# yukiteruono/pbsim3

Measured on AMD Instinct MI355X. Metric: simulated bases/sec, higher is better.
Workload: dtype u8

## Files before the change

pbsim3_amd/csrc/ctx.h:

```cpp
#pragma once
#include <hip/hip_runtime.h>
#include <limits.h>
#include <stdio.h>
#include <stdlib.h>
#include <stdint.h>

#include <algorithm>
#include <condition_variable>
#include <functional>
#include <memory>
#include <mutex>
#include <string>
#include <vector>

#include "../../include/pbsim3_amd.h"
#include "host_tables.h"
#include "kernels.h"

namespace pbsim {
extern thread_local std::string g_err;
int fail(const std::string &m);
}


// ... 55 lines not shown
      return e;
    }
    bytes = want;
    return hipSuccess;
  }
};

using namespace pbsim;

constexpr int kMaxSlots = 6;
constexpr int kPipelineDepth = 2;
static_assert(kPipelineDepth >= 1 && kPipelineDepth <= kMaxSlots, "the pipeline's slots are the first of kMaxSlots");

constexpr size_t kScratchSlack = 64u << 10;
constexpr double kSinkBatchBases = 5.0e9;

constexpr int kDfBuffers = 5;
struct DfLane {
  DevBuf d_df_status, d_df_ctl;
  uint32_t epoch = 0;
  DevBuf d_df_dense[kDfBuffers];
  DevBuf d_df_code;
  HostBuf h_df_total, h_df_out[kDfBuffers];
  hipStream_t stream = nullptr;
  hipStream_t copy_stream = nullptr;
  bool own_streams = false;
  hipStream_t own[2] = {nullptr, nullptr};
  bool pre_valid = false, pre_own_staging = false, pre_elsewhere = false;
  const uint8_t *pre_text = nullptr;
  int64_t pre_n = 0;
  int pre_count = 0;
  hipStream_t lane_stream = nullptr;
  hipEvent_t ev_pre = nullptr;
  hipEvent_t ev_df[kDfBuffers] = {}, ev_cp[kDfBuffers] = {};
  hipEvent_t ev_k0[kDfBuffers] = {}, ev_k1[kDfBuffers] = {};
  std::vector<std::unique_ptr<HostBuf>> arena_blocks;
  std::vector<size_t> arena_fill;
  std::vector<char> arena_touched;
  std::vector<int> arena_idle;
  std::vector<std::pair<const char *, int64_t>> arena_segs;
  size_t arena_bytes() const {
    size_t n = 0;
    for (const auto &b : arena_blocks) n += b->bytes;
    return n;
  }
  void arena_reset() {
    std::fill(arena_fill.begin(), arena_fill.end(), 0);
    arena_segs.clear();
  }
  char *arena_reserve(int64_t n, size_t max_bytes) {
    static const size_t kBlock = getenv("PBSIM_PINNED_BLOCK_KB") && atoll(getenv("PBSIM_PINNED_BLOCK_KB")) > 0
                                     ? (size_t)atoll(getenv("PBSIM_PINNED_BLOCK_KB")) << 10 : (size_t)256u << 20;
    const size_t need = ((size_t)n + 63) & ~(size_t)63;
    for (size_t i = 0; i < arena_blocks.size(); i++) {
      HostBuf &b = *arena_blocks[i];
      if (arena_fill[i] + need <= b.bytes) {
        char *p = (char *)b.p + arena_fill[i];
        arena_fill[i] += need;
        arena_touched[i] = 1;
        arena_segs.emplace_back(p, n);
        return p;
      }
    }
    const size_t want = std::max(kBlock, need);
    if (max_bytes && arena_bytes() + want > max_bytes) return nullptr;
    if (getenv("PBSIM_TRACE")) fprintf(stderr, "[pbsim arena] new block of %zu MB (lane holds %zu MB in %zu blocks)\n", want >> 20, arena_bytes() >> 20, arena_blocks.size());
// ... 208 lines not shown
  hipEvent_t ev_prof_base = nullptr;
  std::vector<std::pair<float, float>> prof_intervals;
  double prof_text_ms = 0, prof_deflate_ms = 0;
  int64_t prof_text_launches = 0, prof_text_in = 0, prof_text_out = 0;
  int64_t prof_deflate_launches = 0, prof_deflate_in = 0, prof_deflate_out = 0;
  std::mutex prof_mu;
};

namespace pbsim {
RefDesc current_ref(const pbsim_ctx *c);
int64_t quota_of(const pbsim_ctx *c, int64_t ref_len);
int walk_begin(pbsim_ctx *c, const RefDesc &ref, int64_t first_read, int64_t n_reads, int64_t truncate_remaining, bool chain = false,
               double factor = 0.0 );
double scratch_factor_of(const pbsim_ctx *c);
int chain_end_finalize(pbsim_ctx *c, int64_t len_total_before, pbsim_batch_info *out);
int chain_reads_for(const pbsim_ctx *c, int64_t ref_len, int64_t remaining);
constexpr int kChainReads = 6;
int64_t batch_capacity_for(const pbsim_ctx *c, int64_t ref_len);
int finalize_cut(pbsim_ctx *c, int64_t len_total_before, pbsim_batch_info *out);
int finalize_text(pbsim_ctx *c, pbsim_batch_info *info);
int finalize_uncut(pbsim_ctx *c, pbsim_batch_info *out);
std::string sam_header_text(const pbsim_ctx *c, int64_t unit);
std::string truth_bam_header_bytes(const pbsim_ctx *c, int64_t ref_len);
int truth_bam_check_names(const pbsim_ctx *c);
int account_slot(pbsim_ctx *c, StatsAcc *st);
int account_of(pbsim_ctx *c, Slot &sl, StatsAcc *st);
void stats_add_task(StatsAcc *st, int64_t len_max, bool quality, long len, long nsub, long nins, long ndel, double qsum,
                    std::vector<double> *values);
void stats_finish(const StatsAcc &st, const pbsim_params &p, int64_t ref_len, pbsim_stats *o);
int stats_merge(StatsAcc *st, const pbsim_params &p, const pbsim_comm *comm, int64_t *extra, int n_extra);
int deflate_prelaunch(pbsim_ctx *c, Slot &sl, bool want_read, bool want_maf);
int deflate_pieces(pbsim_ctx *c, DfLane &lane, const uint8_t *d_text, int64_t n,
                   const std::function<int(const char *, int64_t)> &consume,
                   const std::function<char *(int64_t)> *place = nullptr);
int ensure_deflate_ready(pbsim_ctx *c);
int ensure_crc_tables(pbsim_ctx *c);
int prepare_enqueue(pbsim_ctx *c, uint8_t *d_seq, DevBuf &hp, DevBuf &tiles, DevBuf &flags, int64_t len, hipStream_t stream);
int ensure_tables(pbsim_ctx *c, bool hp11);
inline bool has_quality(const pbsim_ctx *c) { return c->p.method == PBSIM_METHOD_QS || c->p.method == PBSIM_METHOD_SAMPLE; }
}
```

pbsim3_amd/csrc/deflate_host.cpp:

```cpp
#include <hip/hip_runtime.h>
#include <limits.h>
#include <math.h>
#include <stdio.h>
#include <stdlib.h>
#include <string.h>

#include <algorithm>
#include <chrono>
#include <functional>
#include <memory>
#include <string>
#include <thread>
#include <vector>

#include "ctx.h"
#include "engine_internal.h"
#include "unit_io.h"

extern "C" {

extern "C++" {
namespace {

int ensure_deflate_tables(pbsim_ctx *c) {
// ... 76 lines not shown
  launch_deflate_table(d_text, n, reinterpret_cast<uint32_t *>(sl.d_df_code.as<uint8_t>() + DF_TABLE_BYTES), sl.d_df_code.p, sl.stream);
  if (!sl.ev_df[0]) {
    for (int i = 0; i < kDfBuffers; i++) {
      HIP_OK(hipEventCreateWithFlags(&sl.ev_df[i], hipEventDisableTiming));
      HIP_OK(hipEventCreateWithFlags(&sl.ev_cp[i], hipEventDisableTiming));
      HIP_OK(hipEventCreate(&sl.ev_k0[i]));
      HIP_OK(hipEventCreate(&sl.ev_k1[i]));
    }
  }
  unsigned long long *d_prof = nullptr;
  if (getenv("PBSIM_DEFLATE_PROF")) {
    HIP_OK(c->d_df_prof.ensure(128));
    HIP_OK(hipMemsetAsync(c->d_df_prof.p, 0, 128, sl.stream));
    d_prof = c->d_df_prof.as<unsigned long long>();
  }
  const int64_t first = std::min<int64_t>(launch_stream ? 1 : g.ahead, g.n_pieces);
  for (int64_t j = 0; j < first; j++)
    if (!df_launch_piece(c, sl, g, d_text, n, j, false, own_staging, d_prof)) return PBSIM_FAILED;
  sl.pre_count = (int)first;
  sl.pre_text = d_text;
  sl.pre_n = n;
  sl.pre_own_staging = own_staging;
  sl.pre_valid = true;
  sl.pre_elsewhere = launch_stream != nullptr;
  if (launch_stream) {
    if (!sl.ev_pre) HIP_OK(hipEventCreateWithFlags(&sl.ev_pre, hipEventDisableTiming));
    HIP_OK(hipEventRecord(sl.ev_pre, launch_stream));
  }
  return PBSIM_SUCCEEDED;
}

template <class F>
int deflate_stream(pbsim_ctx *c, DfLane &sl, const uint8_t *d_text, int64_t n, F &&consume,
                   const std::function<char *(int64_t)> *place = nullptr) {
  if (n <= 0) return PBSIM_SUCCEEDED;
  const bool prelaunched = sl.pre_valid && sl.pre_text == d_text && sl.pre_n == n && sl.pre_own_staging == (place == nullptr);
  sl.pre_valid = false;
  if (!prelaunched && !df_begin(c, sl, d_text, n, place == nullptr, nullptr)) return PBSIM_FAILED;
  sl.pre_valid = false;
  if (sl.pre_elsewhere) {
    sl.stream = sl.lane_stream;
    HIP_OK(hipStreamWaitEvent(sl.stream, sl.ev_pre, 0));
    sl.pre_elsewhere = false;
  }
  const DfGeom g = df_geom(n);
  const int64_t n_pieces = g.n_pieces;
  const int ahead = g.ahead, nbuf = g.nbuf;
  unsigned long long *d_prof = getenv("PBSIM_DEFLATE_PROF") ? c->d_df_prof.as<unsigned long long>() : nullptr;
  const bool trace = getenv("PBSIM_DEFLATE_TRACE") != nullptr;
  const auto now = []() { return std::chrono::duration<double, std::milli>(std::chrono::steady_clock::now().time_since_epoch()).count(); };
  double t_kernel = 0, t_copy = 0, t_consume = 0, t_begin = now();
  int64_t out_bytes = 0;
  std::vector<std::pair<hipEvent_t, hipEvent_t>> tev;
  bool used[kDfBuffers] = {false};
  int64_t *h_total = reinterpret_cast<int64_t *>(sl.h_df_total.p);
  auto launch = [&](int64_t j) -> int {
    return df_launch_piece(c, sl, g, d_text, n, j, used[(int)(j % nbuf)], place == nullptr, d_prof);
  };
  for (int64_t j = sl.pre_count; j < std::min<int64_t>(ahead, n_pieces); j++)
    if (!launch(j)) return PBSIM_FAILED;
  const char *prev_ptr = nullptr;
  int64_t prev_bytes = 0;
  int prev_buf = 0;
  for (int64_t k = 0; k < n_pieces; k++) {
    const int b = (int)(k % nbuf);
    const double t0 = now();
    HIP_OK(hipEventSynchronize(sl.ev_df[b]));
    t_kernel += now() - t0;
    const int64_t total = h_total[2 * b + 1];
    if ((uint64_t)h_total[2 * b] >> 32) return fail("deflate: a workgroup's look-back gave up waiting for its predecessors");
    out_bytes += total;
    {
      float ms = 0;
      if (hipEventElapsedTime(&ms, sl.ev_k0[b], sl.ev_k1[b]) == hipSuccess) {
        std::lock_guard<std::mutex> lk(c->prof_mu);
        c->prof_deflate_ms += ms;
        c->prof_deflate_launches++;
        c->prof_deflate_in += g.len(k, n);
        c->prof_deflate_out += total;
      }
    }
    char *dst = place ? (*place)(total) : (char *)sl.h_df_out[b].p;
    if (!dst) return fail("deflate: no room for a compressed piece");
    HIP_OK(hipStreamWaitEvent(sl.copy_stream, sl.ev_df[b], 0));
    if (trace) {
      hipEvent_t e0 = nullptr, e1 = nullptr;
      HIP_OK(hipEventCreate(&e0));
      HIP_OK(hipEventCreate(&e1));
      tev.emplace_back(e0, e1);
      HIP_OK(hipEventRecord(e0, sl.copy_stream));
    }
    HIP_OK(hipMemcpyAsync(dst, sl.d_df_dense[b].p, (size_t)total, hipMemcpyDeviceToHost, sl.copy_stream));
    if (trace) HIP_OK(hipEventRecord(tev.back().second, sl.copy_stream));
    HIP_OK(hipEventRecord(sl.ev_cp[b], sl.copy_stream));
    used[b] = true;
    if (prev_bytes) {
      const double t1 = now();
      HIP_OK(hipEventSynchronize(sl.ev_cp[prev_buf]));
      const double t2 = now();
      if (!consume(prev_ptr, prev_bytes)) return PBSIM_FAILED;
      t_copy += t2 - t1;
      t_consume += now() - t2;
    }
    prev_ptr = dst;
    prev_bytes = total;
    prev_buf = b;
    if (k + ahead < n_pieces && !launch(k + ahead)) return PBSIM_FAILED;
  }
  if (prev_bytes) {
    const double t1 = now();
    HIP_OK(hipEventSynchronize(sl.ev_cp[prev_buf]));
    const double t2 = now();
    if (!consume(prev_ptr, prev_bytes)) return PBSIM_FAILED;
    t_copy += t2 - t1;
    t_consume += now() - t2;
  }
  if (trace) {
    double t_link = 0, t_span = 0;
    float ms = 0;
    for (auto &e : tev) {
      if (hipEventElapsedTime(&ms, e.first, e.second) == hipSuccess) t_link += ms;
    }
    if (!tev.empty() && hipEventElapsedTime(&ms, tev.front().first, tev.back().second) == hipSuccess) t_span = ms;
    for (auto &e : tev) {
      (void)hipEventDestroy(e.first);
      (void)hipEventDestroy(e.second);
    }
    fprintf(stderr,
            "[deflate] %.1f MB -> %.1f MB in %.1f ms: waited %.1f ms for kernels, %.1f ms for copies, %.1f ms in the consumer; copies: "
            "%.1f ms on the engine within a span of %.1f ms (%.1f GB/s while copying)\n",
            n / 1e6, out_bytes / 1e6, now() - t_begin, t_kernel, t_copy, t_consume, t_link, t_span, t_link > 0 ? out_bytes / t_link / 1e6 : 0.0);
  }
  if (d_prof) {
    unsigned long long t[16];
    HIP_OK(hipMemcpy(t, d_prof, 128, hipMemcpyDeviceToHost));
    const double nch = (double)((n + DF_CHUNK - 1) / DF_CHUNK);
    static const char *names[7] = {"stage", "crc", "sizes+scan", "header", "tokens", "trailer", "store"};
    fprintf(stderr, "[deflate prof] %.0f chunks; us per chunk (lane 0):", nch);
    for (int i = 0; i < 7; ++i) fprintf(stderr, " %s %.1f", names[i], t[i] / nch / 100);
    fprintf(stderr, "\n");
  }
  return PBSIM_SUCCEEDED;
}

int deflate_to_host(pbsim_ctx *c, DfLane &sl, const uint8_t *d_text, int64_t n, char *host_dst, int64_t cap,
                    int64_t *out_bytes) {
  int64_t written = 0;
  const int ok = deflate_stream(c, sl, d_text, n, [&](const char *z, int64_t k) {
    if (written + k > cap) return fail("deflate: output buffer too small");
    memcpy(host_dst + written, z, (size_t)k);
    written += k;
    return PBSIM_SUCCEEDED;
  });
  *out_bytes = written;
  return ok;
}

}
}

extern "C++" int pbsim::deflate_pieces(pbsim_ctx *c, DfLane &lane, const uint8_t *d_text, int64_t n,
                                       const std::function<int(const char *, int64_t)> &consume,
                                       const std::function<char *(int64_t)> *place) {
  return deflate_stream(c, lane, d_text, n, consume, place);
}
extern "C++" int pbsim::ensure_deflate_ready(pbsim_ctx *c) {
  for (auto &lane : c->df_streams)
    for (hipStream_t &st : lane)
      if (!st) HIP_OK(hipStreamCreateWithFlags(&st, hipStreamNonBlocking));
  return ensure_deflate_tables(c);
}
extern "C++" int pbsim::ensure_crc_tables(pbsim_ctx *c) { return ensure_deflate_tables(c); }
extern "C++" int pbsim::deflate_prelaunch(pbsim_ctx *c, Slot &sl, bool want_read, bool want_maf) {
  const pbsim_batch_info &bi = sl.b_info;
  if (want_read && bi.read_text_bytes > 0 && !df_begin(c, sl.df[0], sl.d_read_text.as<uint8_t>(), bi.read_text_bytes, true, sl.stream))
    return PBSIM_FAILED;
  if (want_maf && bi.maf_text_bytes > 0 && !df_begin(c, sl.df[1], sl.d_maf_text.as<uint8_t>(), bi.maf_text_bytes, true, sl.stream))
    return PBSIM_FAILED;
  return PBSIM_SUCCEEDED;
}

int pbsim_set_deflate(pbsim_ctx *c, int on) {
  if (!c) return fail("bad argument");
  c->deflate = on & 3;
  c->deflate_parallel = (on & 4) != 0;
  return PBSIM_SUCCEEDED;
}

int64_t pbsim_deflate_bound(int64_t n) {
  if (n <= 0) return 0;
  return n + ((n + DF_CHUNK - 1) / DF_CHUNK) * 31;
}

int pbsim_batch_fetch_deflated(pbsim_ctx *c, char *read_gz, int64_t read_cap, char *maf_gz, int64_t maf_cap,
                               int64_t *read_gz_bytes, int64_t *maf_gz_bytes) {
  if (!c || !c->s().b_finalized) return fail("pbsim_batch_fetch_deflated: no finalized batch");
  NEED_DEVICE(c);
// ... 93 lines not shown
```

pbsim3_amd/csrc/engine.cpp:

```cpp
#include <hip/hip_runtime.h>
#include <limits.h>
#include <math.h>
#include <stdio.h>
#include <stdlib.h>
#include <string.h>

#include <algorithm>
#include <chrono>
#include <functional>
#include <memory>
#include <string>
#include <thread>
#include <unordered_map>
#include <vector>

#include "ctx.h"
#include "engine_internal.h"
#include "unit_io.h"
#include "philox.h"

namespace pbsim {
thread_local std::string g_err;
int fail(const std::string &m) {
  g_err = m;
// ... 234 lines not shown
    (void)hipEventCreate(&sl.ev2);
    (void)hipEventCreate(&sl.ev3);
  }
  if (const char *sf = getenv("PBSIM_SCRATCH_FACTOR")) {
    if (atof(sf) >= 1.0) {
      c->scratch_factor = std::min(2.0, atof(sf));
      c->scratch_factor_fixed = true;
    }
  }
  const char *mb = getenv("PBSIM_SCRATCH_MB");
  c->scratch_budget = (mb && atoll(mb) > 0) ? atoll(mb) * (1LL << 20) : (8LL << 30);
  c->scratch_auto = !(mb && atoll(mb) > 0);
  return c.release();
}

void pbsim_destroy(pbsim_ctx *c) {
  if (!c) return;
  if (c->device >= 0) (void)hipSetDevice(c->device);
  if (c->stream) (void)hipStreamSynchronize(c->stream);
  for (Slot &sl : c->slots) {
    if (sl.stream) (void)hipStreamSynchronize(sl.stream);
    if (sl.ev0) (void)hipEventDestroy(sl.ev0);
    if (sl.ev1) (void)hipEventDestroy(sl.ev1);
    if (sl.ev2) (void)hipEventDestroy(sl.ev2);
    if (sl.ev3) (void)hipEventDestroy(sl.ev3);
    if (sl.stream) (void)hipStreamDestroy(sl.stream);
    for (DfLane &L : sl.df) {
      for (int i = 0; i < kDfBuffers; i++) {
        if (L.ev_df[i]) (void)hipEventDestroy(L.ev_df[i]);
        if (L.ev_cp[i]) (void)hipEventDestroy(L.ev_cp[i]);
        if (L.ev_k0[i]) (void)hipEventDestroy(L.ev_k0[i]);
        if (L.ev_k1[i]) (void)hipEventDestroy(L.ev_k1[i]);
      }
      for (hipStream_t &st : L.own)
        if (st) (void)hipStreamDestroy(st);
    }
    if (sl.walk_stream) (void)hipStreamDestroy(sl.walk_stream);
    if (sl.ev_prep) (void)hipEventDestroy(sl.ev_prep);
    if (sl.coop_stream) (void)hipStreamDestroy(sl.coop_stream);
    if (sl.ev_coop) (void)hipEventDestroy(sl.ev_coop);
    if (sl.ev_text) (void)hipEventDestroy(sl.ev_text);
    if (sl.ev_t0) (void)hipEventDestroy(sl.ev_t0);
    if (sl.ev_c0) (void)hipEventDestroy(sl.ev_c0);
    if (sl.ev_c1) (void)hipEventDestroy(sl.ev_c1);
    if (sl.ev_t1) (void)hipEventDestroy(sl.ev_t1);
  }
  for (auto &lane : c->df_streams)
    for (hipStream_t &st : lane)
      if (st) (void)hipStreamDestroy(st);
  if (c->ev_prof_base) (void)hipEventDestroy(c->ev_prof_base);
  if (c->prefetch_stream) (void)hipStreamDestroy(c->prefetch_stream);
  if (c->sq_stream) (void)hipStreamDestroy(c->sq_stream);
  for (Slot &sl : c->slots) {
    if (sl.ev_sq_walk) (void)hipEventDestroy(sl.ev_sq_walk);
    if (sl.ev_sq_done) (void)hipEventDestroy(sl.ev_sq_done);
  }
  if (c->stream) (void)hipStreamDestroy(c->stream);
  delete c;
}

int pbsim_load_errhmm(pbsim_ctx *c, const char *path) {
  if (!c || !path) return fail("pbsim_load_errhmm: bad argument");
  std::unique_ptr<ErrModel> m(new ErrModel);
  std::string e;
  if (!parse_errhmm(path, m.get(), &e)) return fail(e);
  c->err = std::move(m);
  c->class_tables_dirty = true;
  c->coop_wg_errhmm[0] = c->coop_wg_errhmm[1] = 0;
  return PBSIM_SUCCEEDED;
}

int pbsim_load_qshmm(pbsim_ctx *c, const char *path) {
  if (!c || !path) return fail("pbsim_load_qshmm: bad argument");
  std::unique_ptr<QsModel> m(new QsModel);
  std::string e;
  if (!parse_qshmm(path, m.get(), &e)) return fail(e);
  c->qs = std::move(m);
  c->class_tables_dirty = true;
  c->coop_wg_errhmm[0] = c->coop_wg_errhmm[1] = 0;
  return PBSIM_SUCCEEDED;
}

int pbsim_release_pools(pbsim_ctx *c) {
  if (!c) return fail("bad argument");
  NEED_DEVICE(c);
  HIP_OK(hipSetDevice(c->device));
  for (Slot &sl : c->slots) {
    if (sl.b_enqueued) return fail("pbsim_release_pools: a batch is in flight");
    if (sl.stream) HIP_OK(hipStreamSynchronize(sl.stream));
  }
  HIP_OK(hipDeviceSynchronize());
  for (Slot &sl : c->slots) {
    sl.d_scratch.release();
    sl.d_read_text.release();
    sl.d_maf_text.release();
    for (DfLane &L : sl.df) {
      for (DevBuf &b : L.d_df_dense) b.release();
      L.arena_release();
    }
    sl.b_walked = sl.b_finalized = false;
  }
  {
    std::lock_guard<std::mutex> lk(c->job_mu);
    c->job_spare.clear();
  }
  return PBSIM_SUCCEEDED;
}

int pbsim_set_scratch_bytes(pbsim_ctx *c, int64_t bytes) {
  if (!c || bytes < (1 << 20)) return fail("pbsim_set_scratch_bytes: bad argument");
  c->scratch_budget = bytes;
  c->scratch_auto = false;
  return PBSIM_SUCCEEDED;
}

int pbsim_add_hp_census(pbsim_ctx *c, const uint8_t *seq, int64_t len) {
  if (!c || !seq || len < 1) return fail("pbsim_add_hp_census: bad argument");
  NEED_DEVICE(c);
  HIP_OK(hipSetDevice(c->device));
  HIP_OK(c->d_seq_own.ensure((size_t)len + 64));
  HIP_OK(hipMemcpyAsync(c->d_seq_own.p, seq, (size_t)len, hipMemcpyHostToDevice, c->stream));
  HIP_OK(hipMemsetAsync(c->d_seq_own.as<uint8_t>() + len, 0, 64, c->stream));
// ... 1201 lines not shown
```

pbsim3_amd/csrc/job.cpp:

```cpp
#include <math.h>
#include <stdio.h>
#include <stdlib.h>
#include <string.h>

#include <algorithm>
#include <atomic>
#include <chrono>
#include <condition_variable>
#include <deque>
#include <future>
#include <mutex>
#include <thread>

#include "ctx.h"

using namespace pbsim;

namespace {

double now_us() {
  return std::chrono::duration<double, std::micro>(std::chrono::steady_clock::now().time_since_epoch()).count();
}

constexpr double kMinBatchBases = 2.0e9;
constexpr int kRoundsPerRecord = 4;

struct Rec {
  RefDesc ref;
  int64_t quota = 0, len_total = 0, next_read = 1, spec_read = 1;
  double spec_total = 0;
  int64_t cap = 0;
  bool bulk_done = false;
  bool done = false;
  int owner = -1;
  int tail_slot = -1;
  bool tail_waiting = false;
  int64_t read_off = 0, maf_off = 0;
  int64_t tail_read = 0, tail_maf = 0;
  StatsAcc st;
  bool merged = false;
};

struct Round {
  int rec, slot;
  int64_t first, n_per;
  double mean;
  bool clear;
// ... 248 lines not shown
      if (r.slot == s) return true;
    for (const Rec &r : recs)
      if (r.tail_slot == s) return true;
    return false;
  }
  static constexpr int kTailSlot = kMaxSlots - 2;
  int free_slot() const {
    for (int s = 0; s < kTailSlot; s++)
      if (!slot_busy(s)) return s;
    return -1;
  }
  int free_tail_slot() const {
    for (int s = kTailSlot; s < kMaxSlots; s++)
      if (!slot_busy(s)) return s;
    return -1;
  }
  int bulk_in_flight() const { return (int)fifo.size(); }
  int acquire_slot() {
    const double t0 = now_us();
    for (;;) {
      const int s = free_slot();
      if (s >= 0) {
        bd_slot_wait += now_us() - t0;
        return s;
      }
      std::unique_lock<std::mutex> lk(worker.mu);
      worker.cv_idle.wait_for(lk, std::chrono::milliseconds(2));
    }
  }

  void drop_round(const Round &r) {
    c->cur = r.slot;
    (void)hipStreamSynchronize(c->s().stream);
    c->s().b_enqueued = false;
  }
  void drop_rounds_of(int rec) {
    for (auto it = fifo.begin(); it != fifo.end();) {
      if (it->rec == rec) {
        drop_round(*it);
        it = fifo.erase(it);
      } else {
        ++it;
      }
    }
  }
  void drop_everything(bool failing = true) {
    if (failing) {
      giving_up = true;
      { std::lock_guard<std::mutex> lk(out_mu); }
      out_cv.notify_all();
    }
    worker.drain();
    tail_worker.drain();
    for (const Round &r : fifo) drop_round(r);
    fifo.clear();
    for (Rec &r : recs)
      if (r.tail_slot >= 0) {
        c->cur = r.tail_slot;
        (void)hipStreamSynchronize(c->s().stream);
        c->s().b_enqueued = false;
        r.tail_slot = -1;
      }
  }

  size_t arena_max = 0;
  bool wants_text() const { return sink && (sink->on_read_text || sink->on_maf_text); }
  bool deflated() const { return wants_text() && c->deflate == 3; }

  int fetch_plain(Slot &sl) {
    const pbsim_batch_info &bi = sl.b_info;
    const bool want_r = sink->on_read_text && bi.read_text_bytes, want_m = sink->on_maf_text && bi.maf_text_bytes;
    if (want_r) {
      HIP_OK(sl.h_read_text.ensure((size_t)bi.read_text_bytes + 16));
      HIP_OK(hipMemcpyAsync(sl.h_read_text.p, sl.d_read_text.p, (size_t)bi.read_text_bytes, hipMemcpyDeviceToHost, sl.stream));
    }
    if (want_m) {
      HIP_OK(sl.h_maf_text.ensure((size_t)bi.maf_text_bytes + 16));
      HIP_OK(hipMemcpyAsync(sl.h_maf_text.p, sl.d_maf_text.p, (size_t)bi.maf_text_bytes, hipMemcpyDeviceToHost, sl.stream));
    }
    HIP_OK(hipStreamSynchronize(sl.stream));
    return PBSIM_SUCCEEDED;
  }
  int call_sink(int which, int64_t unit, const char *text, int64_t bytes, int64_t at) {
    std::lock_guard<std::mutex> lk(sink_mu[which]);
    return (which == 0 ? sink->on_read_text : sink->on_maf_text)(sink->user, unit, text, bytes, at);
  }
  int sink_plain(Slot &sl, int64_t unit, int64_t read_at, int64_t maf_at) {
    const pbsim_batch_info &bi = sl.b_info;
    if (sink->on_read_text && bi.read_text_bytes && !call_sink(0, unit, (const char *)sl.h_read_text.p, bi.read_text_bytes, read_at))
      return fail("sink aborted (read text)");
    if (sink->on_maf_text && bi.maf_text_bytes && !call_sink(1, unit, (const char *)sl.h_maf_text.p, bi.maf_text_bytes, maf_at))
      return fail("sink aborted (MAF text)");
    return PBSIM_SUCCEEDED;
  }
  template <class F>
  int both_lanes(Slot &sl, F &&lane) {
    const pbsim_batch_info &bi = sl.b_info;
    if (c->deflate_parallel && bi.read_text_bytes && bi.maf_text_bytes && sink->on_read_text && sink->on_maf_text) {
      int ok_read = PBSIM_SUCCEEDED;
      std::string err_read;
      std::thread t([&]() {
        (void)hipSetDevice(c->device);
        ok_read = lane(0);
        if (!ok_read) err_read = g_err;
      });
      const int ok_maf = lane(1);
      t.join();
      if (!ok_read) return fail(err_read);
      return ok_maf;
    }
    return lane(0) && lane(1);
  }
  int stream_deflated(Slot &sl, int64_t unit, int64_t read_at, int64_t maf_at, int64_t *read_gz, int64_t *maf_gz) {
    const pbsim_batch_info &bi = sl.b_info;
    *read_gz = *maf_gz = 0;
    return both_lanes(sl, [&](int which) -> int {
      const bool is_read = which == 0;
      const int64_t n = is_read ? bi.read_text_bytes : bi.maf_text_bytes;
      auto cb = is_read ? sink->on_read_text : sink->on_maf_text;
      int64_t *sent = is_read ? read_gz : maf_gz;
      const int64_t base = is_read ? read_at : maf_at;
      const uint8_t *d = is_read ? sl.d_read_text.as<uint8_t>() : sl.d_maf_text.as<uint8_t>();
      if (!cb || n == 0) return PBSIM_SUCCEEDED;
      return deflate_pieces(c, sl.df[which], d, n, [&](const char *z, int64_t k) {
        if (!call_sink(which, unit, z, k, base + *sent)) return fail(is_read ? "sink aborted (read text)" : "sink aborted (MAF text)");
        *sent += k;
        return PBSIM_SUCCEEDED;
      });
    });
  }
  int arena_fill(Slot &sl, int64_t *read_gz, int64_t *maf_gz) {
    const pbsim_batch_info &bi = sl.b_info;
    *read_gz = *maf_gz = 0;
    return both_lanes(sl, [&](int which) -> int {
      DfLane &L = sl.df[which];
      L.arena_reset();
      const int64_t n = which == 0 ? bi.read_text_bytes : bi.maf_text_bytes;
      auto cb = which == 0 ? sink->on_read_text : sink->on_maf_text;
      if (!cb || n == 0) return PBSIM_SUCCEEDED;
      const uint8_t *d = which == 0 ? sl.d_read_text.as<uint8_t>() : sl.d_maf_text.as<uint8_t>();
      bool oom = false;
      const std::function<char *(int64_t)> place = [&](int64_t k) -> char * {
        char *p = L.arena_reserve(k, arena_max);
        if (!p) oom = true;
        return p;
      };
      if (!deflate_pieces(c, L, d, n, [](const char *, int64_t) { return PBSIM_SUCCEEDED; }, &place))
        return oom ? fail("out of pinned host memory for a compressed batch (PBSIM_PINNED_ARENA_MB bounds a lane's arena)") : PBSIM_FAILED;
      int64_t tot = 0;
      for (const auto &sg : L.arena_segs) tot += sg.second;
      (which == 0 ? *read_gz : *maf_gz) = tot;
      return PBSIM_SUCCEEDED;
    });
  }
  int arena_flush(Slot &sl, int64_t unit, int64_t read_at, int64_t maf_at) {
    return both_lanes(sl, [&](int which) -> int {
      int64_t at = which == 0 ? read_at : maf_at;
      for (const auto &sg : sl.df[which].arena_segs) {
        if (!call_sink(which, unit, sg.first, sg.second, at)) return fail(which == 0 ? "sink aborted (read text)" : "sink aborted (MAF text)");
        at += sg.second;
      }
      sl.df[which].arena_segs.clear();
      return PBSIM_SUCCEEDED;
    });
  }

  void submit_stage1(Delivery *d) {
    d->stage1 = std::make_shared<std::promise<int>>();
    d->stage1_done = d->stage1->get_future();
    if (!d->mine) {
      d->stage1->set_value(PBSIM_SUCCEEDED);
      return;
    }
    delivering[d->slot] = true;
    Slot *sl = &c->slots[d->slot];
    Rec *R = &recs[(size_t)d->rec];
    auto prom = d->stage1;
    int64_t *sizes = d->sizes;
    const int64_t read_at = R->read_off, maf_at = R->maf_off;
    std::atomic<int> *out = &rec_out[(size_t)d->rec], *bulk = &rec_bulk[(size_t)d->rec];
// ... 249 lines not shown
    const double t0 = now_us();
    progress(4, rec);
    if (!stats_merge(&R.st, c->p, multi ? comm : nullptr, extra, 3)) return PBSIM_FAILED;
    bd_merge += now_us() - t0;
    if (!tail_ok) return fail(tail_err);
    if (!check_worker()) return PBSIM_FAILED;
    if (extra[2]) {
      peer_failed = true;
      return fail("another rank of the job failed");
    }
    R.merged = R.done = true;
    pbsim_stats st;
    stats_finish(R.st, c->p, R.ref.len, &st);
    c->st = R.st;
    c->st.blocks.clear();
    R.st = StatsAcc();
    if (sink && sink->on_record_done &&
        !sink->on_record_done(sink->user, recs[(size_t)rec].ref.unit, &st, R.read_off + extra[0], R.maf_off + extra[1]))
      return fail("sink aborted (record done)");
    return PBSIM_SUCCEEDED;
  }

  int begin_round(int rec) {
    Rec &R = recs[(size_t)rec];
    const double remaining = (double)R.quota - R.spec_total;
    int64_t n_total = (int64_t)(1.005 * remaining / mean) + 64;
    if (remaining <= 0) n_total = 64;
    int64_t n_per = std::min<int64_t>((n_total + W - 1) / W, R.cap);
    if (rounds < 2) n_per = std::min<int64_t>(n_per, std::max<int64_t>(64, (int64_t)((double)R.cap * (rounds == 0 ? 0.2 : 0.5))));
    n_per = std::max<int64_t>(n_per, 1);
    if (!collect(rec)) return PBSIM_FAILED;
    const int s = acquire_slot();
    c->cur = s;
    const double tb = now_us();
    if (trace) fprintf(stderr, "[pbsim job r%d] begin rec %d first=%lld n_per=%lld\n", rank, rec + 1, (long long)R.spec_read, (long long)n_per);
    if (!walk_begin(c, R.ref, R.spec_read + (int64_t)rank * n_per, n_per, -1)) return PBSIM_FAILED;
    bd_begin += now_us() - tb;
    const double after = R.spec_total + (double)W * (double)n_per * mean;
    static const char *force_clear = getenv("PBSIM_JOB_CLEAR");
    const bool clear = force_clear ? atoi(force_clear) != 0
                                   : (double)R.quota - after > 0.04 * (double)W * (double)n_per * mean + 2.0 * (double)std::min<int64_t>(c->p.len_max, R.ref.len);
    fifo.push_back(Round{rec, s, R.spec_read, n_per, mean, clear});
    R.spec_read += (int64_t)W * n_per;
    R.spec_total += (double)W * (double)n_per * mean;
    reads_walked += n_per;
    rounds++;
    return PBSIM_SUCCEEDED;
  }

  static constexpr int kMsg = 8;
  int process_round() {
    const Round rd = fifo.front();
    fifo.pop_front();
    Rec &R = recs[(size_t)rd.rec];
    c->cur = rd.slot;
    const double t0 = now_us();
    int64_t pass0 = 0, code = 0;
    std::string my_err;
    if (!pbsim_batch_walk_end(c, &pass0)) {
      my_err = g_err;
      code = (my_err.rfind("scratch budget exceeded", 0) == 0 && rd.n_per > 1) ? 1 : 2;
    }
    if (wfailed) code = 2;
    const double t1 = now_us();
    bd_wait_walk += t1 - t0;
    for (size_t r = 0; r < recs.size(); r++)
      if ((recs[r].tail_slot >= 0 || recs[r].tail_waiting) && !tail_poll((int)r, false)) return PBSIM_FAILED;
    c->cur = rd.slot;
    const int64_t max_raw = c->s().b_max_raw;
    pbsim_batch_info bi;
    memset(&bi, 0, sizeof bi);
    int fin_ok = PBSIM_SUCCEEDED;
    double t_fin = 0;
    std::vector<int64_t> A, B;
    int64_t msg[kMsg] = {pass0, code, max_raw, 0, 0, 0, 0, 0};
    bool c_applied = false;
    if (rd.clear) {
      if (code == 0) {
        const double tf = now_us();
        fin_ok = finalize_uncut(c, &bi) && finalize_text(c, &bi);
        if (!fin_ok) my_err = g_err;
        t_fin += now_us() - tf;
      }
      msg[3] = fin_ok ? 0 : 1;
      if (pending) {
        msg[4] = 1;
        if (!wait_pending(&msg[5])) return PBSIM_FAILED;
      }
      progress(6, rd.rec, rd.first, rd.n_per);
      if (!gather(msg, kMsg, &A)) return PBSIM_FAILED;
      c_applied = true;
    } else {
      progress(1, rd.rec, rd.first, rd.n_per);
      if (!gather(msg, kMsg, &A)) return PBSIM_FAILED;
    }
    int64_t worst = 0, pass0_sum = 0, before = R.len_total, raw_all = 0, bad_fin = 0;
    for (int q = 0; q < W; q++) {
      worst = std::max(worst, A[(size_t)q * kMsg + 1]);
      pass0_sum += A[(size_t)q * kMsg];
      raw_all = std::max(raw_all, A[(size_t)q * kMsg + 2]);
      bad_fin += A[(size_t)q * kMsg + 3];
      if (q < rank) before += A[(size_t)q * kMsg];
    }
    if (c_applied && worst != 2 && !apply_pending(A, kMsg, 5, true)) return PBSIM_FAILED;
    if (worst == 2 || (worst == 0 && bad_fin)) {
      drop_everything();
      if (wfailed) return check_worker();
      if (code != 2 && fin_ok) peer_failed = true;
      return fail(code == 2 || !fin_ok ? my_err : "another rank of the job failed");
    }
    if (worst == 1) {
      if (!complete_pending()) return PBSIM_FAILED;
      drop_everything(false);
      for (Rec &r : recs) {
        r.spec_read = r.next_read;
        r.spec_total = (double)r.len_total;
        r.cap = std::min(r.cap, std::max<int64_t>(1, rd.n_per / 2));
        if (r.owner == rank && r.bulk_done && !r.done && !tail_begin(r)) return PBSIM_FAILED;
      }
      return PBSIM_SUCCEEDED;
    }
    const bool untouched = R.len_total + pass0_sum + raw_all <= R.quota;
    B.assign((size_t)W * kMsg, 0);
    if (rd.clear && untouched) {
      int64_t lt = R.len_total;
      for (int q = 0; q < W; q++) {
        lt += A[(size_t)q * kMsg];
        B[(size_t)q * kMsg] = rd.n_per;
        B[(size_t)q * kMsg + 2] = lt;
      }
      bi.len_total_after = before + pass0;
      c->s().b_info.len_total_after = bi.len_total_after;
    } else {
      const double tf = now_us();
      fin_ok = (untouched ? finalize_uncut(c, &bi) : finalize_cut(c, before, &bi)) && finalize_text(c, &bi);
      if (!fin_ok) my_err = g_err;
      if (untouched) c->s().b_info.len_total_after = bi.len_total_after = before + pass0;
      t_fin += now_us() - tf;
      if (rd.clear) n_clear_missed++;
      int64_t msgB[kMsg] = {bi.n_final, bi.need_truncated_read, bi.len_total_after, fin_ok ? 0 : 1, 0, 0, 0, 0};
      if (!rd.clear && pending) {
        msgB[4] = 1;
        if (!wait_pending(&msgB[5])) return PBSIM_FAILED;
        c_applied = true;
      }
      progress(rd.clear ? 2 : 7, rd.rec, rd.first, rd.n_per);
      if (!gather(msgB, kMsg, &B)) return PBSIM_FAILED;
      int64_t bad_b = 0;
      for (int q = 0; q < W; q++) bad_b += B[(size_t)q * kMsg + 3];
      if (!rd.clear && !bad_b && !apply_pending(B, kMsg, 5, true)) return PBSIM_FAILED;
      if (bad_b) {
        drop_everything();
        if (fin_ok) peer_failed = true;
        return fail(fin_ok ? "another rank of the job failed" : my_err);
      }
    }
    bd_finalize += t_fin;
    const double t2 = now_us();
    int cut = -1;
    for (int q = 0; q < W && cut < 0; q++)
      if (B[(size_t)q * kMsg] < rd.n_per) cut = q;
    const int last_valid = cut < 0 ? W - 1 : cut;
    const bool mine = rank <= last_valid && bi.n_final > 0;
    if (!c_applied && !complete_pending(true)) return PBSIM_FAILED;
    pending.reset(new Delivery);
    ++rec_rounds_open[(size_t)rd.rec];
    pending->slot = rd.slot;
    pending->rec = rd.rec;
    pending->mine = mine;
    pending->n_per = rd.n_per;
    submit_stage1(pending.get());
    if (!account_deferred()) return PBSIM_FAILED;
    if (mine) {
      reads_delivered += bi.n_final;
      bases += bi.bases;
      ref_bases += bi.ref_bases;
      maf_columns += bi.maf_columns;
    }
    const double t3 = now_us();
    const double n_round = (double)W * (double)rd.n_per;
    R.spec_total += (double)pass0_sum - n_round * rd.mean;
    if (n_round >= 1000) {
      const double measured = (double)pass0_sum / n_round;
      for (Round &pr : fifo) {
        recs[(size_t)pr.rec].spec_total += (double)W * (double)pr.n_per * (measured - pr.mean);
        pr.mean = measured;
      }
      mean = measured;
    }
    if (cut < 0) {
      R.next_read += (int64_t)W * rd.n_per;
      R.len_total = B[(size_t)(W - 1) * kMsg + 2];
    } else {
      R.next_read += (int64_t)cut * rd.n_per + B[(size_t)cut * kMsg];
      R.len_total = B[(size_t)cut * kMsg + 2];
      R.spec_read = R.next_read;
      R.spec_total = (double)R.len_total;
      if (B[(size_t)cut * kMsg + 1] && R.len_total < R.quota) {
        R.owner = cut;
        R.bulk_done = true;
      }
    }
    if (R.len_total >= R.quota) R.bulk_done = true;
    if (R.bulk_done) {
      drop_rounds_of(rd.rec);
      if (rank == R.owner) {
        if (!tail_begin(R)) return PBSIM_FAILED;
      } else {
        R.done = true;
      }
    }
    if (trace)
      fprintf(stderr,
              "[pbsim job r%d] t=%.1f ms rec %d round first=%lld n=%lldx%d %s final=%lld cut=%d wait_walk=%.1f finalize=%.1f handover=%.1f "
              "comm=%.1f ms\n",
              rank, (t0 - t_start) / 1e3, rd.rec + 1, (long long)rd.first, (long long)rd.n_per, W,
              rd.clear ? (untouched ? "clear" : "clear-missed") : "cutting", (long long)bi.n_final, cut, (t1 - t0) / 1e3, t_fin / 1e3,
              (t3 - t2) / 1e3, comm_us / 1e3);
    return PBSIM_SUCCEEDED;
  }

  int run() {
    const int n = (int)recs.size();
    int merged = 0;
    worker.start(c->device);
    tail_worker.start(c->device);
    for (;;) {
      if (!check_worker()) return PBSIM_FAILED;
      const int open_max = std::max(2, interleave);
      while (bulk_in_flight() < depth) {
        int cand = -1;
        const int hi = std::min(n, merged + open_max);
        double best = 2.0;
        for (int r = merged; r < hi; r++) {
          const Rec &R = recs[(size_t)r];
          if (R.bulk_done || (double)R.quota - R.spec_total <= 0) continue;
          if (interleave <= 1) {
            cand = r;
            break;
          }
          const double f = R.spec_total / (double)std::max<int64_t>(1, R.quota);
          if (f < best) {
            best = f;
            cand = r;
          }
        }
        if (cand < 0) {
          for (int r = merged; r < hi && cand < 0; r++) {
            bool has = false;
            for (const Round &pr : fifo) has |= pr.rec == r;
            if (!recs[(size_t)r].bulk_done && !has) cand = r;
          }
          if (cand >= 0) n_topup++;
        }
        if (cand < 0) {
          if (hi >= n) break;
          if (!recs[(size_t)merged].bulk_done) break;
          if (!finish_record(merged)) return PBSIM_FAILED;
          merged++;
          continue;
        }
        if (!begin_round(cand)) return PBSIM_FAILED;
      }
// ... 375 lines not shown
  if (J.sink && (J.sink->on_read_text || J.sink->on_maf_text)) target = std::min(target, kSinkBatchBases);
  if (c->scratch_auto) {
    size_t free_b = 0, total_b = 0;
    HIP_OK(hipMemGetInfo(&free_b, &total_b));
    if (streaming) {
      std::lock_guard<std::mutex> lk(c->job_mu);
      std::vector<int64_t> spare;
      for (auto &sp : c->job_spare) spare.push_back(sp->len);
      size_t pending = 0, lines_max = 0;
      for (size_t i = 0; i < n; i++) {
        if (i < c->job_records.size()) {
          free_b += (size_t)(2 * lens[i] + 192);
        }
        auto it = std::find(spare.begin(), spare.end(), lens[i]);
        if (it != spare.end() && i >= c->job_records.size()) {
          spare.erase(it);
          continue;
        }
        pending += (size_t)(2 * lens[i] + 192) + (size_t)(lens[i] / 1024 + 64) * 16;
        lines_max = std::max(lines_max, (size_t)(lens[i] + lens[i] / 40 + 64));
      }
      if (c->d_lines.bytes > 0 && lines_max > c->d_lines.bytes) pending += lines_max - c->d_lines.bytes;
      free_b = free_b > pending ? free_b - pending : 0;
    }
    size_t held = 0, held_text = 0;
    for (Slot &sl : c->slots) {
      held += sl.d_scratch.bytes;
      held_text += sl.d_read_text.bytes + sl.d_maf_text.bytes;
    }
    {
      const double text_per_base = 1.125 * ((P > 1 ? (c->bam_output ? 5.8 : 8.4) : 4.25) + (c->truth_bam ? 0.2 : 0.0));
      const double scratch_per_base = (double)regions * sf * 1.12 * 1.08 + 0.1;
      const bool delivering_text = J.sink && (J.sink->on_read_text || J.sink->on_maf_text);
      const double slots_used = (double)J.depth + (delivering_text ? 2.0 : 1.0);
      const char *ff = getenv("PBSIM_JOB_FIT");
      const double fit = (ff ? atof(ff) : 0.75) * (double)(free_b + held + held_text) / (slots_used * (text_per_base + scratch_per_base));
      target = std::min(target, std::max(fit, 1.0e8));
    }
    const double mean_len = std::max(1.0, c->hdr.mean_len);
    const double want = (target / P / mean_len) * P * ((double)regions * (sf * mean_len + kScratchPad) * 1.12 + 64.0) * 1.08 + (64 << 20);
    const double share = std::min(48.0 * (1LL << 30), 0.14 * (double)(free_b + held));
    const int64_t auto_b = (int64_t)std::max(256.0 * (1 << 20), std::min(want, share));
    if ((double)auto_b > 1.10 * (double)c->scratch_budget || c->scratch_budget > 2 * auto_b) c->scratch_budget = auto_b;
  }
  if (const char *tr = getenv("PBSIM_JOB_TARGET_RANKS")) {
    std::vector<double> v;
    for (const char *q = tr; *q;) {
      char *e = nullptr;
      v.push_back(strtod(q, &e));
      if (e == q) break;
      q = *e == ',' ? e + 1 : e;
    }
    if (!v.empty() && v[(size_t)J.rank % v.size()] > 0) target = v[(size_t)J.rank % v.size()];
  }
  std::vector<int64_t> agree(n + 1);
  agree[0] = c->scratch_budget;
  J.progress(5, -1);
  if (multi) {
    if (!comm->all_reduce_i64(comm->user, agree.data(), 1, PBSIM_OP_MIN)) return fail("pbsim_comm.all_reduce_i64 failed");
    c->scratch_budget = agree[0];
  }
  J.mean = 0.97 * c->hdr.mean_len;
  for (size_t i = 0; i < n; i++) {
    Rec &R = J.recs[i];
    const double m = std::min<double>(c->hdr.mean_len, (double)R.ref.len);
    R.cap = std::max<int64_t>(1, std::min<int64_t>(batch_capacity_for(c, R.ref.len), (int64_t)(1.08 * target / P / m) + 64));
    agree[i + 1] = R.cap;
  }
  if (multi) {
    if (!comm->all_reduce_i64(comm->user, agree.data(), (int64_t)agree.size(), PBSIM_OP_MIN)) return fail("pbsim_comm.all_reduce_i64 failed");
    for (size_t i = 0; i < n; i++) J.recs[i].cap = agree[i + 1];
  }
  J.mean = std::min<double>(J.mean, (double)lens[0]);
  for (Slot &sl : c->slots) sl.b_enqueued = sl.b_walked = sl.b_finalized = false;
  {
    const char *am = getenv("PBSIM_PINNED_ARENA_MB");
    J.arena_max = (size_t)(am && atoll(am) > 0 ? atoll(am) : 16384) << 20;
  }
  int ready = (!J.deflated() || ensure_deflate_ready(c)) ? PBSIM_SUCCEEDED : PBSIM_FAILED;
  if (multi) {
    const std::string keep = g_err;
    int64_t bad = ready ? 0 : 1;
    if (!comm->all_reduce_i64(comm->user, &bad, 1, PBSIM_OP_MAX)) return fail("pbsim_comm.all_reduce_i64 failed");
    if (bad) {
      *settled = true;
      return ready ? fail("another rank of the job failed") : fail(keep);
    }
  } else if (!ready) {
    return PBSIM_FAILED;
  }
  const int keep_lds = c->walk_lds_kb;
  if (J.deflated()) c->walk_lds_kb = std::max(c->walk_lds_kb, 81);
  c->defer_text_sync = true;
  int ok = J.run();
  c->defer_text_sync = false;
  c->walk_lds_kb = keep_lds;
  for (Slot &sl : c->slots)
    if (sl.stream && hipStreamSynchronize(sl.stream) != hipSuccess && ok) ok = fail("hipStreamSynchronize failed at the end of the job");
  if (!ok) {
    const std::string keep = g_err;
    if (multi && !J.peer_failed && comm->abort) comm->abort(comm->user);
    *settled = true;
    J.drop_everything();
    J.worker.finish();
    J.tail_worker.finish();
    g_err = keep;
  }
  for (Slot &sl : c->slots)
    for (DfLane &L : sl.df) L.arena_trim();
  {
    const double wall = now_us() - J.t_start;
    double *b = c->job_breakdown;
    b[0] = wall;
    b[1] = J.bd_wait_walk;
    b[2] = J.bd_finalize;
    b[3] = J.bd_wait_bytes;
    b[4] = J.comm_us;
    b[5] = J.bd_account;
    b[6] = J.bd_tail_block;
    b[7] = J.bd_drain;
    b[8] = J.bd_slot_wait + J.bd_record_wait;
    b[9] = J.bd_merge;
    b[10] = J.bd_begin;
    b[11] = J.bd_tail_steps;
    b[12] = J.bd_worker_busy;
    b[13] = (double)J.n_topup;
    b[14] = (double)J.n_tail_reads;
    b[15] = (double)J.depth;
  }
  c->job_counters[0] = J.reads_walked;
  c->job_counters[1] = J.reads_delivered;
  c->job_counters[2] = J.rounds;
  c->job_counters[3] = J.bases;
  c->job_counters[4] = (int64_t)(now_us() - J.t_start);
  c->job_counters[5] = (int64_t)J.comm_us;
  c->job_counters[6] = J.ref_bases;
  c->job_counters[7] = J.maf_columns;
  return ok;
}

int pbsim_job_run(pbsim_ctx *c, const pbsim_comm *comm, const pbsim_record_sink *sink) {
  if (!c) return fail("bad argument");
// ... 40 lines not shown
```

Measured before the change: 56.34 billion.

## Hand off next round's deflate head launches at the tail of current deflate

Adds a handoff mechanism so that while a lane deflates the tail of one batch, it prelaunches the first pieces of the next finalized batch's text on the same lane stream. This targets idle deflate kernel time between batches. It also adds a lookahead that raises the in-flight depth to two for small rounds, and it budgets one more slot of memory when text is delivered. The cost is extra synchronisation and settle logic, a risk of wasted launches when a round falls behind the cut, and a smaller batch size from the higher slot count.

```diff
diff --git a/pbsim3_amd/csrc/ctx.h b/pbsim3_amd/csrc/ctx.h
--- a/pbsim3_amd/csrc/ctx.h
+++ b/pbsim3_amd/csrc/ctx.h
@@ -111,6 +111,8 @@
   int pre_count = 0;
   hipStream_t lane_stream = nullptr;
   hipEvent_t ev_pre = nullptr;
+  hipEvent_t ev_hand = nullptr;
+  bool hand_open = false;
   hipEvent_t ev_df[kDfBuffers] = {}, ev_cp[kDfBuffers] = {};
   hipEvent_t ev_k0[kDfBuffers] = {}, ev_k1[kDfBuffers] = {};
   std::vector<std::unique_ptr<HostBuf>> arena_blocks;
@@ -385,7 +387,10 @@
 int deflate_prelaunch(pbsim_ctx *c, Slot &sl, bool want_read, bool want_maf);
 int deflate_pieces(pbsim_ctx *c, DfLane &lane, const uint8_t *d_text, int64_t n,
                    const std::function<int(const char *, int64_t)> &consume,
-                   const std::function<char *(int64_t)> *place = nullptr);
+                   const std::function<char *(int64_t)> *place = nullptr, const std::function<bool()> *tail_hook = nullptr);
+int deflate_handoff(pbsim_ctx *c, DfLane &next, int lane_index, const uint8_t *d_text, int64_t n, bool own_staging,
+                    hipEvent_t text_ready);
+int deflate_settle(DfLane &lane);
 int ensure_deflate_ready(pbsim_ctx *c);
 int ensure_crc_tables(pbsim_ctx *c);
 int prepare_enqueue(pbsim_ctx *c, uint8_t *d_seq, DevBuf &hp, DevBuf &tiles, DevBuf &flags, int64_t len, hipStream_t stream);
diff --git a/pbsim3_amd/csrc/deflate_host.cpp b/pbsim3_amd/csrc/deflate_host.cpp
--- a/pbsim3_amd/csrc/deflate_host.cpp
+++ b/pbsim3_amd/csrc/deflate_host.cpp
@@ -132,12 +132,17 @@
 
 template <class F>
 int deflate_stream(pbsim_ctx *c, DfLane &sl, const uint8_t *d_text, int64_t n, F &&consume,
-                   const std::function<char *(int64_t)> *place = nullptr) {
+                   const std::function<char *(int64_t)> *place = nullptr, const std::function<bool()> *tail_hook = nullptr) {
   if (n <= 0) return PBSIM_SUCCEEDED;
   const bool prelaunched = sl.pre_valid && sl.pre_text == d_text && sl.pre_n == n && sl.pre_own_staging == (place == nullptr);
   sl.pre_valid = false;
+  const bool handed = prelaunched && sl.hand_open;
+  if (!prelaunched && !pbsim::deflate_settle(sl)) return PBSIM_FAILED;
   if (!prelaunched && !df_begin(c, sl, d_text, n, place == nullptr, nullptr)) return PBSIM_FAILED;
   sl.pre_valid = false;
+  if (handed && getenv("PBSIM_TRACE"))
+    fprintf(stderr, "[deflate] lane call of %.1f MB found its head handed off (%d pieces launched behind the call in front)\n", n / 1e6,
+            sl.pre_count);
   if (sl.pre_elsewhere) {
     sl.stream = sl.lane_stream;
     HIP_OK(hipStreamWaitEvent(sl.stream, sl.ev_pre, 0));
@@ -150,6 +155,11 @@
   const bool trace = getenv("PBSIM_DEFLATE_TRACE") != nullptr;
   const auto now = []() { return std::chrono::duration<double, std::milli>(std::chrono::steady_clock::now().time_since_epoch()).count(); };
   double t_kernel = 0, t_copy = 0, t_consume = 0, t_begin = now();
+  double t_first_copy = 0, t_last_copy = 0;
+  bool hook_due = false;
+  auto offer_tail = [&]() {
+    if (tail_hook && hook_due && (*tail_hook)()) hook_due = false;
+  };
   int64_t out_bytes = 0;
   std::vector<std::pair<hipEvent_t, hipEvent_t>> tev;
   bool used[kDfBuffers] = {false};
@@ -159,6 +169,8 @@
   };
   for (int64_t j = sl.pre_count; j < std::min<int64_t>(ahead, n_pieces); j++)
     if (!launch(j)) return PBSIM_FAILED;
+  hook_due = n_pieces <= ahead;
+  offer_tail();
   const char *prev_ptr = nullptr;
   int64_t prev_bytes = 0;
   int prev_buf = 0;
@@ -190,6 +202,7 @@
       tev.emplace_back(e0, e1);
       HIP_OK(hipEventRecord(e0, sl.copy_stream));
     }
+    if (k == 0) t_first_copy = now();
     HIP_OK(hipMemcpyAsync(dst, sl.d_df_dense[b].p, (size_t)total, hipMemcpyDeviceToHost, sl.copy_stream));
     if (trace) HIP_OK(hipEventRecord(tev.back().second, sl.copy_stream));
     HIP_OK(hipEventRecord(sl.ev_cp[b], sl.copy_stream));
@@ -206,15 +219,19 @@
     prev_bytes = total;
     prev_buf = b;
     if (k + ahead < n_pieces && !launch(k + ahead)) return PBSIM_FAILED;
+    if (k + ahead == n_pieces - 1) hook_due = true;
+    offer_tail();
   }
   if (prev_bytes) {
     const double t1 = now();
     HIP_OK(hipEventSynchronize(sl.ev_cp[prev_buf]));
     const double t2 = now();
+    t_last_copy = t2;
     if (!consume(prev_ptr, prev_bytes)) return PBSIM_FAILED;
     t_copy += t2 - t1;
     t_consume += now() - t2;
   }
+  sl.hand_open = false;
   if (trace) {
     double t_link = 0, t_span = 0;
     float ms = 0;
@@ -228,8 +245,10 @@
     }
     fprintf(stderr,
             "[deflate] %.1f MB -> %.1f MB in %.1f ms: waited %.1f ms for kernels, %.1f ms for copies, %.1f ms in the consumer; copies: "
-            "%.1f ms on the engine within a span of %.1f ms (%.1f GB/s while copying)\n",
-            n / 1e6, out_bytes / 1e6, now() - t_begin, t_kernel, t_copy, t_consume, t_link, t_span, t_link > 0 ? out_bytes / t_link / 1e6 : 0.0);
+            "%.1f ms on the engine within a span of %.1f ms (%.1f GB/s while copying); first copy enqueued at %.3f, last copy "
+            "complete at %.3f ms%s%s\n",
+            n / 1e6, out_bytes / 1e6, now() - t_begin, t_kernel, t_copy, t_consume, t_link, t_span, t_link > 0 ? out_bytes / t_link / 1e6 : 0.0,
+            t_first_copy, t_last_copy, sl.own_streams ? " (chain lane)" : "", handed ? " (head handed off)" : "");
   }
   if (d_prof) {
     unsigned long long t[16];
@@ -261,8 +280,27 @@
 
 extern "C++" int pbsim::deflate_pieces(pbsim_ctx *c, DfLane &lane, const uint8_t *d_text, int64_t n,
                                        const std::function<int(const char *, int64_t)> &consume,
-                                       const std::function<char *(int64_t)> *place) {
-  return deflate_stream(c, lane, d_text, n, consume, place);
+                                       const std::function<char *(int64_t)> *place, const std::function<bool()> *tail_hook) {
+  return deflate_stream(c, lane, d_text, n, consume, place, tail_hook);
+}
+extern "C++" int pbsim::deflate_handoff(pbsim_ctx *c, DfLane &next, int lane_index, const uint8_t *d_text, int64_t n,
+                                        bool own_staging, hipEvent_t text_ready) {
+  hipStream_t st = c->df_streams[lane_index][0];
+  if (!st || next.own_streams || next.hand_open || n <= 0) return fail("deflate_handoff: bad argument");
+  if (!next.ev_hand) HIP_OK(hipEventCreateWithFlags(&next.ev_hand, hipEventDisableTiming));
+  HIP_OK(hipStreamWaitEvent(st, text_ready, 0));
+  const int ok = df_begin(c, next, d_text, n, own_staging, nullptr);
+  if (!ok) next.pre_valid = false;
+  next.hand_open = true;
+  HIP_OK(hipEventRecord(next.ev_hand, st));
+  return ok;
+}
+extern "C++" int pbsim::deflate_settle(DfLane &lane) {
+  if (!lane.hand_open) return PBSIM_SUCCEEDED;
+  lane.pre_valid = false;
+  HIP_OK(hipEventSynchronize(lane.ev_hand));
+  lane.hand_open = false;
+  return PBSIM_SUCCEEDED;
 }
 extern "C++" int pbsim::ensure_deflate_ready(pbsim_ctx *c) {
   for (auto &lane : c->df_streams)
diff --git a/pbsim3_amd/csrc/engine.cpp b/pbsim3_amd/csrc/engine.cpp
--- a/pbsim3_amd/csrc/engine.cpp
+++ b/pbsim3_amd/csrc/engine.cpp
@@ -290,6 +290,8 @@
         if (L.ev_k0[i]) (void)hipEventDestroy(L.ev_k0[i]);
         if (L.ev_k1[i]) (void)hipEventDestroy(L.ev_k1[i]);
       }
+      (void)deflate_settle(L);
+      if (L.ev_hand) (void)hipEventDestroy(L.ev_hand);
       for (hipStream_t &st : L.own)
         if (st) (void)hipStreamDestroy(st);
     }
@@ -346,6 +348,8 @@
   for (Slot &sl : c->slots) {
     if (sl.b_enqueued) return fail("pbsim_release_pools: a batch is in flight");
     if (sl.stream) HIP_OK(hipStreamSynchronize(sl.stream));
+    for (DfLane &L : sl.df)
+      if (!deflate_settle(L)) return PBSIM_FAILED;
   }
   HIP_OK(hipDeviceSynchronize());
   for (Slot &sl : c->slots) {
diff --git a/pbsim3_amd/csrc/handoff.h b/pbsim3_amd/csrc/handoff.h
--- /dev/null
+++ b/pbsim3_amd/csrc/handoff.h
@@ -0,0 +1,48 @@
+#pragma once
+#include <stdint.h>
+
+#include <mutex>
+
+namespace pbsim {
+
+struct HandoffNext {
+  int slot = -1;
+  const void *text[2] = {nullptr, nullptr};
+  int64_t bytes[2] = {0, 0};
+  void *ev_text = nullptr;
+};
+
+class Handoff {
+ public:
+  void publish(const HandoffNext &d) {
+    std::lock_guard<std::mutex> lk(mu_);
+    d_ = d;
+    up_ = true;
+    taken_[0] = taken_[1] = false;
+  }
+  template <class F>
+  bool take(int lane, F &&run) {
+    std::lock_guard<std::mutex> lk(mu_);
+    if (!up_) return false;
+    if (!taken_[lane]) {
+      taken_[lane] = true;
+      run(d_);
+    }
+    return true;
+  }
+  unsigned withdraw() {
+    std::lock_guard<std::mutex> lk(mu_);
+    const unsigned t = up_ ? (unsigned)taken_[0] | ((unsigned)taken_[1] << 1) : 0u;
+    up_ = false;
+    taken_[0] = taken_[1] = false;
+    return t;
+  }
+
+ private:
+  std::mutex mu_;
+  bool up_ = false;
+  bool taken_[2] = {false, false};
+  HandoffNext d_;
+};
+
+}
diff --git a/pbsim3_amd/csrc/job.cpp b/pbsim3_amd/csrc/job.cpp
--- a/pbsim3_amd/csrc/job.cpp
+++ b/pbsim3_amd/csrc/job.cpp
@@ -13,6 +13,7 @@
 #include <thread>
 
 #include "ctx.h"
+#include "handoff.h"
 
 using namespace pbsim;
 
@@ -327,6 +328,7 @@
   void drop_round(const Round &r) {
     c->cur = r.slot;
     (void)hipStreamSynchronize(c->s().stream);
+    (void)settle_slot(r.slot);
     c->s().b_enqueued = false;
   }
   void drop_rounds_of(int rec) {
@@ -356,6 +358,45 @@
         c->s().b_enqueued = false;
         r.tail_slot = -1;
       }
+  }
+
+  Handoff handoff;
+  bool handoff_on = false;
+  bool lookahead = false;
+  int64_t n_handed = 0, n_handed_void = 0;
+  void publish_next(int slot) {
+    const Slot &sl = c->slots[slot];
+    if (!handoff_on || sl.b_info.n_final <= 0) return;
+    HandoffNext d;
+    d.slot = slot;
+    d.text[0] = sink->on_read_text ? sl.d_read_text.p : nullptr;
+    d.text[1] = sink->on_maf_text ? sl.d_maf_text.p : nullptr;
+    d.bytes[0] = sl.b_info.read_text_bytes;
+    d.bytes[1] = sl.b_info.maf_text_bytes;
+    d.ev_text = sl.ev_text;
+    handoff.publish(d);
+  }
+  unsigned withdraw_next() {
+    if (!handoff_on) return 0;
+    const unsigned took = handoff.withdraw();
+    n_handed += (took & 1) + (took >> 1);
+    return took;
+  }
+  int settle_slot(int slot) {
+    for (DfLane &L : c->slots[slot].df) {
+      if (L.hand_open) n_handed_void++;
+      if (!deflate_settle(L)) return PBSIM_FAILED;
+    }
+    return PBSIM_SUCCEEDED;
+  }
+  std::function<bool()> tail_hook(int which) {
+    return [this, which]() -> bool {
+      return handoff.take(which, [&](const HandoffNext &d) {
+        if (!d.text[which] || d.bytes[which] <= 0) return;
+        (void)deflate_handoff(c, c->slots[d.slot].df[which], which, (const uint8_t *)d.text[which], d.bytes[which], !multi,
+                              (hipEvent_t)d.ev_text);
+      });
+    };
   }
 
   size_t arena_max = 0;
@@ -417,11 +458,12 @@
       const int64_t base = is_read ? read_at : maf_at;
       const uint8_t *d = is_read ? sl.d_read_text.as<uint8_t>() : sl.d_maf_text.as<uint8_t>();
       if (!cb || n == 0) return PBSIM_SUCCEEDED;
+      const std::function<bool()> hook = tail_hook(which);
       return deflate_pieces(c, sl.df[which], d, n, [&](const char *z, int64_t k) {
         if (!call_sink(which, unit, z, k, base + *sent)) return fail(is_read ? "sink aborted (read text)" : "sink aborted (MAF text)");
         *sent += k;
         return PBSIM_SUCCEEDED;
-      });
+      }, nullptr, handoff_on ? &hook : nullptr);
     });
   }
   int arena_fill(Slot &sl, int64_t *read_gz, int64_t *maf_gz) {
@@ -440,7 +482,8 @@
         if (!p) oom = true;
         return p;
       };
-      if (!deflate_pieces(c, L, d, n, [](const char *, int64_t) { return PBSIM_SUCCEEDED; }, &place))
+      const std::function<bool()> hook = tail_hook(which);
+      if (!deflate_pieces(c, L, d, n, [](const char *, int64_t) { return PBSIM_SUCCEEDED; }, &place, handoff_on ? &hook : nullptr))
         return oom ? fail("out of pinned host memory for a compressed batch (PBSIM_PINNED_ARENA_MB bounds a lane's arena)") : PBSIM_FAILED;
       int64_t tot = 0;
       for (const auto &sg : L.arena_segs) tot += sg.second;
@@ -756,12 +799,13 @@
     if (!collect(rec)) return PBSIM_FAILED;
     const int s = acquire_slot();
     c->cur = s;
+    if (!settle_slot(s)) return PBSIM_FAILED;
     const double tb = now_us();
     if (trace) fprintf(stderr, "[pbsim job r%d] begin rec %d first=%lld n_per=%lld\n", rank, rec + 1, (long long)R.spec_read, (long long)n_per);
     if (!walk_begin(c, R.ref, R.spec_read + (int64_t)rank * n_per, n_per, -1)) return PBSIM_FAILED;
     bd_begin += now_us() - tb;
     const double after = R.spec_total + (double)W * (double)n_per * mean;
-    static const char *force_clear = getenv("PBSIM_JOB_CLEAR");
+    const char *force_clear = getenv("PBSIM_JOB_CLEAR");
     const bool clear = force_clear ? atoi(force_clear) != 0
                                    : (double)R.quota - after > 0.04 * (double)W * (double)n_per * mean + 2.0 * (double)std::min<int64_t>(c->p.len_max, R.ref.len);
     fifo.push_back(Round{rec, s, R.spec_read, n_per, mean, clear});
@@ -778,6 +822,10 @@
     fifo.pop_front();
     Rec &R = recs[(size_t)rd.rec];
     c->cur = rd.slot;
+    struct Withdraw {
+      Job *j;
+      ~Withdraw() { (void)j->withdraw_next(); }
+    } withdraw_at_exit{this};
     const double t0 = now_us();
     int64_t pass0 = 0, code = 0;
     std::string my_err;
@@ -804,6 +852,7 @@
         const double tf = now_us();
         fin_ok = finalize_uncut(c, &bi) && finalize_text(c, &bi);
         if (!fin_ok) my_err = g_err;
+        else publish_next(rd.slot);
         t_fin += now_us() - tf;
       }
       msg[3] = fin_ok ? 0 : 1;
@@ -857,8 +906,10 @@
       c->s().b_info.len_total_after = bi.len_total_after;
     } else {
       const double tf = now_us();
-      fin_ok = (untouched ? finalize_uncut(c, &bi) : finalize_cut(c, before, &bi)) && finalize_text(c, &bi);
+      fin_ok = (!withdraw_next() || settle_slot(rd.slot)) && (untouched ? finalize_uncut(c, &bi) : finalize_cut(c, before, &bi)) &&
+               finalize_text(c, &bi);
       if (!fin_ok) my_err = g_err;
+      else publish_next(rd.slot);
       if (untouched) c->s().b_info.len_total_after = bi.len_total_after = before + pass0;
       t_fin += now_us() - tf;
       if (rd.clear) n_clear_missed++;
@@ -887,6 +938,11 @@
     const int last_valid = cut < 0 ? W - 1 : cut;
     const bool mine = rank <= last_valid && bi.n_final > 0;
     if (!c_applied && !complete_pending(true)) return PBSIM_FAILED;
+    const unsigned handed = withdraw_next();
+    if (trace && handoff_on)
+      fprintf(stderr, "[pbsim job r%d] t=%.1f ms rec %d hand-off: %s%s%s\n", rank, (now_us() - t_start) / 1e3, rd.rec + 1,
+              handed == 0 ? "no lane took the round" : (handed == 3 ? "both lanes' heads launched" : "one lane's head launched"),
+              handed ? " behind the round in front" : "", handed && !mine ? " (void: the block is behind the cut)" : "");
     pending.reset(new Delivery);
     ++rec_rounds_open[(size_t)rd.rec];
     pending->slot = rd.slot;
@@ -952,7 +1008,12 @@
     for (;;) {
       if (!check_worker()) return PBSIM_FAILED;
       const int open_max = std::max(2, interleave);
-      while (bulk_in_flight() < depth) {
+      auto depth_now = [&]() {
+        if (!lookahead || depth != 1 || fifo.size() != 1) return depth;
+        const Round &r = fifo.front();
+        return 4 * r.n_per <= recs[(size_t)r.rec].cap ? 2 : 1;
+      };
+      while (bulk_in_flight() < depth_now()) {
         int cand = -1;
         const int hi = std::min(n, merged + open_max);
         double best = 2.0;
@@ -1394,7 +1455,7 @@
       const double text_per_base = 1.125 * ((P > 1 ? (c->bam_output ? 5.8 : 8.4) : 4.25) + (c->truth_bam ? 0.2 : 0.0));
       const double scratch_per_base = (double)regions * sf * 1.12 * 1.08 + 0.1;
       const bool delivering_text = J.sink && (J.sink->on_read_text || J.sink->on_maf_text);
-      const double slots_used = (double)J.depth + (delivering_text ? 2.0 : 1.0);
+      const double slots_used = (double)J.depth + (delivering_text ? 3.0 : 1.0);
       const char *ff = getenv("PBSIM_JOB_FIT");
       const double fit = (ff ? atof(ff) : 0.75) * (double)(free_b + held + held_text) / (slots_used * (text_per_base + scratch_per_base));
       target = std::min(target, std::max(fit, 1.0e8));
@@ -1454,6 +1515,13 @@
   const int keep_lds = c->walk_lds_kb;
   if (J.deflated()) c->walk_lds_kb = std::max(c->walk_lds_kb, 81);
   c->defer_text_sync = true;
+  {
+    const char *ho = getenv("PBSIM_JOB_HANDOFF");
+    J.handoff_on = J.deflated() && c->deflate_parallel && !(ho && atoi(ho) == 0);
+    const char *la = getenv("PBSIM_JOB_LOOKAHEAD");
+    J.lookahead = delivers && !(la && atoi(la) == 0);
+  }
+  if (J.trace) fprintf(stderr, "[pbsim job r%d] entered at %.3f ms, round loop at %.3f ms\n", J.rank, J.t_start / 1e3, now_us() / 1e3);
   int ok = J.run();
   c->defer_text_sync = false;
   c->walk_lds_kb = keep_lds;
@@ -1468,8 +1536,14 @@
     J.tail_worker.finish();
     g_err = keep;
   }
+  (void)J.withdraw_next();
+  for (int s = 0; s < kMaxSlots; s++)
+    if (!J.settle_slot(s) && ok) ok = PBSIM_FAILED;
   for (Slot &sl : c->slots)
     for (DfLane &L : sl.df) L.arena_trim();
+  if (J.trace)
+    fprintf(stderr, "[pbsim job r%d] returns at %.3f ms; hand-off %s: %lld lane heads launched at a tail, %lld of them never delivered\n",
+            J.rank, now_us() / 1e3, J.handoff_on ? "on" : "off", (long long)J.n_handed, (long long)J.n_handed_void);
   {
     const double wall = now_us() - J.t_start;
     double *b = c->job_breakdown;
```

New measurement: 58.25 billion, median of 6. +3.4%, better.
